# mitchelldurbincs/GeneralsReinforcementLearning

Measured on AMD Instinct MI355X. Metric: env steps/sec (whole node), 20x20 4P fog-on; state bit-exact vs the C restatement of the Go engine (the reference's own test vectors pass on both), higher is better.
Workload: dtype int32

## Files before the change

generalsreinforcementlearning_amd/csrc/gvec_device.hpp:

```cpp
#pragma once
#include <hip/hip_runtime.h>
#include <stdint.h>

#include "../../include/generals_vec.h"

extern "C" __device__ int gvec_llvm_writelane(int value, int lane, int vdst_in) __asm("llvm.amdgcn.writelane.i32");

#ifndef GVEC_NT
#define GVEC_NT 14
#endif
#define GVEC_NT_MASK 2
#define GVEC_NT_PLANE 4
#define GVEC_NT_ARMY 8
#ifndef GVEC_SC1
#define GVEC_SC1 1
#endif

namespace gvec {

typedef uint32_t u32x4 __attribute__((ext_vector_type(4)));

template <typename T>
__device__ __forceinline__ T ld_stream(const T* p) {
  if constexpr ((GVEC_NT & 1) != 0) return __builtin_nontemporal_load(p);
  return *p;
}
__device__ __forceinline__ void st_through(uint32_t* p, uint32_t v) { asm volatile("global_store_dword %0, %1, off sc1 nt" : : "v"(p), "v"(v) : "memory"); }
__device__ __forceinline__ void st_through(uint16_t* p, uint16_t v) {
  asm volatile("global_store_short %0, %1, off sc1 nt" : : "v"(p), "v"((uint32_t)v) : "memory");
}
__device__ __forceinline__ void st_through(float* p, float v) { asm volatile("global_store_dword %0, %1, off sc1 nt" : : "v"(p), "v"(v) : "memory"); }
__device__ __forceinline__ void st_through(u32x4* p, u32x4 v) {
  asm volatile("global_store_dwordx4 %0, %1, off sc1 nt\n\ts_nop 1" : : "v"(p), "v"(v) : "memory");
}
template <int CLASS, typename T>
__device__ __forceinline__ void st_stream(T* p, T v) {
  if constexpr ((GVEC_NT & CLASS) != 0) {
    if constexpr (GVEC_SC1 != 0) st_through(p, v);
    else __builtin_nontemporal_store(v, p);
  } else {
    *p = v;
  }
}

constexpr int HDR_DW = 24;
enum : int {
  H_TURN = 0,
  H_DIMS = 1,
  H_STATUS = 2,
  H_EPISODE = 3,
  H_ARMYCNT = 4,
  H_GIDX = 12,
  H_RECIPW = 20,
  H_CNT_STEPS = 21,
  H_CNT_ABORT = 22,
  H_CNT_DONE = 23
};
constexpr uint32_t HF_DONE = 1u, HF_FOG = 2u, HF_WIDE = 4u;
constexpr uint32_t HF_SETUP = 8u;
constexpr uint32_t HF_SYNC = 16u;
constexpr uint32_t HF_VSMALL = 32u;
constexpr uint32_t HF_LDIFF = 128u;
constexpr uint32_t HF_FEWSPECIAL = 64u;

template <int MAXP>
struct Planes {
  static constexpr int OWN = 0, VIS = MAXP, CHG = 2 * MAXP, VCH = 2 * MAXP + 1, GT1 = 2 * MAXP + 2,
                       GEN = 2 * MAXP + 3, CITY = 2 * MAXP + 4, MTN = 2 * MAXP + 5, VALID = 2 * MAXP + 6, NCOL0 = 2 * MAXP + 7,
                       NCOLL = 2 * MAXP + 8, OK = 2 * MAXP + 9 , LST = 2 * MAXP + 13,
                       COUNT = 3 * MAXP + 13, MUTABLE = 2 * MAXP + 3, SHARED = 13 ;
};

constexpr uint32_t KF_AGENT = 1u;
constexpr uint32_t KF_EMIT = 2u;
constexpr uint32_t KF_AUTORESET = 4u;
constexpr uint32_t KF_LMVALID = 16u;

struct StepArgs {
  uint32_t* hdr;
  uint32_t* rows;
  uint32_t* army16;
  int32_t* army32;
  const gvec_action* actions;
  gvec_action* actions_out;
  int32_t* err;
  uint32_t* legal;
  const uint32_t* zeros;
  const uint32_t* pool_hdr;
  const uint32_t* pool_rows;
  const uint32_t* pool_army16;
  const int32_t* pool_army32;
  int32_t num_envs, fd, row_dw, mask_dw, pool_size;
  int32_t pstride;
  int32_t prod_general, prod_city, prod_normal, interval;
  uint32_t interval_magic;
  int32_t turns, invalid_permille;
  uint32_t agent_noop, agent_half;
  uint32_t flags, seed_lo, seed_hi, pool_seed_lo, pool_seed_hi;
  uint32_t seed_base, pool_seed_base;
  int32_t env_base;
};

struct ArmyRef {
  uint32_t* n;
  int32_t* w;
};
struct ArmyCRef {
  const uint32_t* n;
  const int32_t* w;
  __device__ __forceinline__ ArmyCRef(const uint32_t* n_, const int32_t* w_) : n(n_), w(w_) {}
  __device__ __forceinline__ ArmyCRef(const ArmyRef& r) : n(r.n), w(r.w) {}
};
template <int NSLOT>
__device__ __forceinline__ ArmyRef army_ref(uint32_t* a16, int32_t* a32, int env) {
  return ArmyRef{a16 + (size_t)env * (NSLOT * 32), a32 + (size_t)env * (NSLOT * 64)};
}
template <int NSLOT>
__device__ __forceinline__ ArmyCRef army_cref(const uint32_t* a16, const int32_t* a32, int env) {
  return ArmyCRef(a16 + (size_t)env * (NSLOT * 32), a32 + (size_t)env * (NSLOT * 64));
}
template <int NSLOT>
__device__ __forceinline__ void army_load_narrow(int32_t (&army)[NSLOT], const uint32_t* n) {
  const int lane = (int)(threadIdx.x & 63u);
#pragma unroll
  for (int k = 0; k < NSLOT / 2; ++k) {
    const uint32_t w = ld_stream(n + 64 * k + lane);
    army[2 * k] = (int32_t)(w & 0xFFFFu);
    army[2 * k + 1] = (int32_t)(w >> 16);
  }
  if constexpr ((NSLOT & 1) != 0) army[NSLOT - 1] = (int32_t)ld_stream(reinterpret_cast<const uint16_t*>(n + 64 * (NSLOT / 2)) + lane);
}
template <int NSLOT>
__device__ __forceinline__ void army_load_wide(int32_t (&army)[NSLOT], const int32_t* w) {
  const int lane = (int)(threadIdx.x & 63u);
#pragma unroll
  for (int s = 0; s < NSLOT; ++s) army[s] = w[64 * s + lane];
}
template <int NSLOT>
__device__ __forceinline__ bool army_fits_narrow(const int32_t (&army)[NSLOT]) {
  uint32_t m = 0u;
#pragma unroll
  for (int s = 0; s < NSLOT; ++s) m |= (uint32_t)army[s];
  return __builtin_amdgcn_ballot_w64(m > 0xFFFFu) == 0ull;
}
template <int NSLOT>
__device__ __forceinline__ void army_store_narrow(const int32_t (&army)[NSLOT], uint32_t* n) {
  const int lane = (int)(threadIdx.x & 63u);
#pragma unroll
  for (int k = 0; k < NSLOT / 2; ++k) st_stream<GVEC_NT_ARMY>(n + 64 * k + lane, (uint32_t)army[2 * k] | ((uint32_t)army[2 * k + 1] << 16));
  if constexpr ((NSLOT & 1) != 0) st_stream<GVEC_NT_ARMY>(reinterpret_cast<uint16_t*>(n + 64 * (NSLOT / 2)) + lane, (uint16_t)army[NSLOT - 1]);
}
template <int NSLOT>
__device__ __forceinline__ void army_store_wide(const int32_t (&army)[NSLOT], int32_t* w) {
  const int lane = (int)(threadIdx.x & 63u);
#pragma unroll
  for (int s = 0; s < NSLOT; ++s) w[64 * s + lane] = army[s];
}

__device__ __forceinline__ int lane_id() { return (int)(threadIdx.x & 63u); }

template <int CTRL, int RM = 0xf, int BM = 0xf>
__device__ __forceinline__ uint32_t dpp0(uint32_t v) {
  return (uint32_t)__builtin_amdgcn_update_dpp(0, (int)v, CTRL, RM, BM, false);
}
__device__ __forceinline__ uint32_t from_prev(uint32_t v) { return dpp0<0x138>(v); }
__device__ __forceinline__ uint32_t from_next(uint32_t v) { return dpp0<0x130>(v); }

__device__ __forceinline__ uint32_t wave_scan_add(uint32_t v) {
// ... 233 lines not shown
```

generalsreinforcementlearning_amd/csrc/gvec_kernels.hip:

```cpp
#include "gvec_launch.hpp"
#include "gvec_packed.hpp"

#include <type_traits>

namespace gvec {

constexpr int WAVES_PER_BLOCK = 4;
#ifdef GYM_PLAYERS_WAVES
#define GYM_PLAYERS_WAVES_OF(NSLOT) GYM_PLAYERS_WAVES
#else
#define GYM_PLAYERS_WAVES_OF(NSLOT) ((NSLOT) <= 7 ? 4 : 3)
#endif

template <int MAXP, int NSLOT>
using Turn = PBoard<MAXP, NSLOT>;

template <int MAXP, int NSLOT>
__device__ __forceinline__ uint32_t agent_sample(const Turn<MAXP, NSLOT>& b, const uint32_t (&m)[Turn<MAXP, NSLOT>::NR][4], uint32_t ek,
                                                 const StepArgs& A) {
  using T = Turn<MAXP, NSLOT>;
  constexpr int NR = T::NR, PPR = T::PPR, ROWL = T::ROWL;
  const int lane = lane_id();
  const uint32_t sbase = ek + (uint32_t)b.turn * 0x9E3779B1u + 0x165667B1u;
  uint32_t mine = 0u;
#pragma unroll
  for (int k = 0; k < NR; ++k) {
    const uint32_t player = (uint32_t)T::lane_player(k);
    const uint32_t h1 = amix(mad24(player, 0x4A7C15u, sbase));
    const uint32_t h2 = amix(h1 ^ 0x68E31DA4u);
    const uint32_t hi16 = h2 >> 16;
    const bool act = b.lane_flag(b.alive, k) && !((h1 & 0xFFFFu) < A.agent_noop);
    const bool half = (h1 >> 16) < A.agent_half;
    const bool inv = A.invalid_permille > 0 && (__umul24(h2 & 0xFFFFu, 1000u) >> 16) < (uint32_t)A.invalid_permille;
    const uint32_t c0 = (uint32_t)__builtin_popcount(m[k][0]), c1 = c0 + (uint32_t)__builtin_popcount(m[k][1]);
    const uint32_t c2 = c1 + (uint32_t)__builtin_popcount(m[k][2]), cnt = c2 + (uint32_t)__builtin_popcount(m[k][3]);
    const uint32_t sc = row_scan_add<ROWL>(cnt);
    const uint32_t total = row_last<ROWL>(sc);
    const uint32_t kk = __umul24(hi16, total) >> 16;
    const uint32_t below = sc - cnt;
    const bool sel = kk >= below && kk < sc;
    const uint32_t r = kk - below;
    const uint32_t d = (r >= c0 ? 1u : 0u) + (r >= c1 ? 1u : 0u) + (r >= c2 ? 1u : 0u);
    const uint32_t base = (d == 0u) ? 0u : (d == 1u) ? c0 : (d == 2u) ? c1 : c2;
    const uint32_t w = (d == 0u) ? m[k][0] : (d == 1u) ? m[k][1] : (d == 2u) ? m[k][2] : m[k][3];
    const uint32_t t_sel = 32u * (uint32_t)T::col() + kth_set_bit(w, r - base);
    const uint32_t pick = row_scan_or<ROWL>(sel ? (t_sel | (d << 10) | 0x8000u) : 0u);
    const uint32_t unchecked = (__umul24(hi16, (uint32_t)b.N) >> 16) | (((h1 >> 8) & 3u) << 10) | 0x8000u;
    const uint32_t fin = inv ? unchecked : pick;
    const bool go = act && (fin & 0x8000u) != 0u;
    const uint32_t out = (fin & 0xFFFu) | (go ? 0x1000u : 0u) | (half ? 0x2000u : 0u);
    const uint32_t got = bperm((((lane % PPR) * ROWL) + ROWL - 1) << 2, out);
    mine = (lane / PPR == k) ? got : mine;
  }
  return mine;
}

template <int MAXP, int NSLOT>
__device__ __forceinline__ void agent_words(const Turn<MAXP, NSLOT>& b, uint32_t mine, uint32_t& alo, uint32_t& ahi) {
  const bool act = lane_id() < MAXP && (mine & 0x1000u) != 0u;
  const int t = (int)(mine & 0x3FFu), d = (int)((mine >> 10) & 3u);
  const int y = (int)(__umul24((uint32_t)t, (uint32_t)b.recipW) >> 16), x = t - (int)__umul24((uint32_t)y, (uint32_t)b.W);
  const int dx = (d == 1) - (d == 3), dy = (d == 2) - (d == 0);
  const uint32_t lo = ((uint32_t)x & 0xFFu) | (((uint32_t)y & 0xFFu) << 8) | (((uint32_t)(x + dx) & 0xFFu) << 16) |
                      (((uint32_t)(y + dy) & 0xFFu) << 24);
  alo = act ? lo : 0u;
  ahi = act ? (GVEC_ACT_VALID | ((mine & 0x2000u) ? GVEC_ACT_HALF : 0u)) : 0u;
}

template <int MAXP, int NSLOT>
__device__ __forceinline__ typename Turn<MAXP, NSLOT>::ActVec agent_actvec(const Turn<MAXP, NSLOT>& b, uint32_t mine, bool may_be_unchecked) {
  typename Turn<MAXP, NSLOT>::ActVec v;
  const bool act = lane_id() < MAXP && (mine & 0x1000u) != 0u;
  const int t = (int)(mine & 0x3FFu), d = (int)((mine >> 10) & 3u);
  uint32_t code = 0u;
  if (may_be_unchecked) {
    const int y = (int)(__umul24((uint32_t)t, (uint32_t)b.recipW) >> 16), x = t - (int)__umul24((uint32_t)y, (uint32_t)b.W);
    const bool off = (d == 0) ? (y == 0) : (d == 1) ? (x == b.W - 1) : (d == 2) ? (y == b.H - 1) : (x == 0);
    code = off ? GVEC_ERR_INVALID_COORDINATES : 0u;
  }
  v.meta = act ? (code | 16u | ((mine & 0x2000u) ? 32u : 0u)) : 0u;
  v.ft = t;
  v.tt = t + ((d == 0) ? -b.W : (d == 1) ? 1 : (d == 2) ? b.W : -1);
  return v;
}

template <typename BT>
__device__ __forceinline__ void load_board(BT& b, const uint32_t* hdr, const uint32_t* rows, const ArmyCRef& army, int fd) {
  b.load_hdr(hdr);
  b.load_army(army);
  b.load_planes(rows, fd);
}
template <bool EARLY = false, typename BT>
__device__ __forceinline__ void load_turn(BT& b, const uint32_t* hdr, const uint32_t* rows, const ArmyCRef& army, int fd, const uint32_t* zeros) {
  if constexpr (EARLY) {
    b.issue_hdr(hdr);
    b.load_planes(rows, fd, zeros);
    b.load_army_narrow(army);
    b.decode_hdr_scalar(hdr);
    b.land();
    b.land_scalars();
    b.spread_shared();
    b.load_lists(rows, fd);
    b.load_army_wide_if_flagged(army);
  } else {
    b.load_hdr(hdr);
    b.load_army(army);
    b.template load_planes<false>(rows, fd, zeros);
  }
}

template <int MAXP, int NSLOT, typename BT>
__device__ __forceinline__ void redeal(BT& b, const StepArgs& A, int env, int fd, int row_dw) {
  const uint32_t episode = b.hdr_get(H_EPISODE) + 1u;
  const uint32_t cs = b.hdr_get(H_CNT_STEPS), ca = b.hdr_get(H_CNT_ABORT), cd = b.hdr_get(H_CNT_DONE);
  const uint32_t hk = fmix32(env_key_of(A.pool_seed_base, (uint32_t)env) ^ (episode * 0x9E3779B1u));
  const int j = (int)__umulhi(hk, (uint32_t)A.pool_size);
  load_turn(b, A.pool_hdr + (size_t)j * HDR_DW, A.pool_rows + (size_t)j * row_dw, army_cref<NSLOT>(A.pool_army16, A.pool_army32, j), fd, A.zeros);
  b.hdr_set(H_EPISODE, episode);
  b.hdr_set(H_CNT_STEPS, cs);
  b.hdr_set(H_CNT_ABORT, ca);
  b.hdr_set(H_CNT_DONE, cd);
}

constexpr int step_waves(int maxp, int nslot) {
  const int ppr = (nslot <= 7) ? 4 : 2;
  const int nr = (maxp + ppr - 1) / ppr;
  const int state = 3 * nr + 13 + nr + nslot + 4 * nr;
  const int need = state + (state + 32 <= 62 ? 32 : 40);
  const int alloc = (need + 7) / 8 * 8;
  const int w = 512 / alloc;
  return w > 8 ? 8 : (w < 2 ? 2 : w);
}

template <int MAXP, int NSLOT, bool AGENT, bool ODD>
__global__ __launch_bounds__(64 * WAVES_PER_BLOCK, step_waves(MAXP, NSLOT)) void step_kernel(StepArgs A) {
  constexpr int FD = 2 * NSLOT - (ODD ? 1 : 0);
  constexpr int ROW_DW = (Planes<MAXP>::COUNT * FD + 3) / 4 * 4;
  __shared__ int32_t army_shadow[WAVES_PER_BLOCK][NSLOT * 64];
  using B = Turn<MAXP, NSLOT>;
  __shared__ uint32_t act_scratch[WAVES_PER_BLOCK][B::ACT_SCRATCH_DW];
  const int wave = (int)(threadIdx.x >> 6), lane = lane_id();
  const int env = uni((int)blockIdx.x * WAVES_PER_BLOCK + wave);
  if (env >= A.num_envs) return;
  bool force_redeal = false;
  if constexpr (!AGENT) {
    const uint32_t f0 = (uint32_t)uni((int)reinterpret_cast<const uint32_t*>(A.actions)[((size_t)env * A.pstride) * 2 + 1]);
    if (f0 & GVEC_ACT_SKIP_ENV) {
      if (A.err && lane == 0) A.err[env] = 0;
      return;
    }
    force_redeal = (f0 & GVEC_ACT_RESET_ENV) != 0u;
  }
  B b;
  b.larmy = army_shadow[wave];
  b.lscr = act_scratch[wave];
  const ArmyRef army_env = army_ref<NSLOT>(A.army16, A.army32, env);
  load_turn<true>(b, A.hdr + (size_t)env * HDR_DW, A.rows + (size_t)env * ROW_DW, army_env, FD, A.zeros);
  b.small = !(b.hflags & HF_WIDE);
  const bool emit = (A.flags & KF_EMIT) != 0u;
  uint32_t m[B::NR][4];
  uint32_t err = 0u;
  bool types_dirty = false, changed = true;
  const bool can_redeal = (A.flags & KF_AUTORESET) && A.pool_size > 0;
  if (AGENT && A.actions_out && (b.hflags & HF_DONE)) {
    if (lane < A.pstride) reinterpret_cast<uint2*>(A.actions_out)[(size_t)env * A.pstride + lane] = make_uint2(0u, 0u);
  }
  if (can_redeal && ((b.hflags & HF_DONE) || force_redeal)) {
    redeal<MAXP, NSLOT>(b, A, env, FD, ROW_DW);
    types_dirty = true;
  } else if (b.hflags & HF_DONE) {
    err = GVEC_ERR_GAME_OVER;
    changed = false;
  } else {
    typename B::ActVec av;
    if constexpr (AGENT) {
      b.template legal_planes<false>(m);
      uint32_t mine = (GVEC_PROFILE_SKIP & 1) ? 0u : agent_sample<MAXP, NSLOT>(b, m, env_key_of(A.seed_base, (uint32_t)env), A);
      if (GVEC_PROFILE_DUP & 64) { b.opaque(); b.template legal_planes<false>(m); }
      if (GVEC_PROFILE_DUP & 1) {
        b.opaque();
#pragma unroll
        for (int d = 0; d < 4; ++d) asm volatile("" : "+v"(m[0][d]));
        const uint32_t again = agent_sample<MAXP, NSLOT>(b, m, env_key_of(A.seed_base, (uint32_t)env), A);
        asm volatile("" : : "v"(again));
      }
      av = agent_actvec<MAXP, NSLOT>(b, mine, A.invalid_permille > 0);
      if (A.actions_out) {
        uint32_t alo, ahi;
        agent_words<MAXP, NSLOT>(b, mine, alo, ahi);
        if (lane < A.pstride) reinterpret_cast<uint2*>(A.actions_out)[(size_t)env * A.pstride + lane] = make_uint2(alo, ahi);
      }
    } else {
      uint32_t alo = 0u, ahi = 0u;
      if (lane < A.pstride) {
        const uint2 w = reinterpret_cast<const uint2*>(A.actions)[(size_t)env * A.pstride + lane];
        alo = w.x;
        ahi = w.y;
      }
      av = b.prevalidate(alo, ahi);
    }
    bool aborted;
    err = b.turn_step(av, A, aborted);
    if (!(GVEC_PROFILE_SKIP & 32)) b.refresh_gt1();
    if (GVEC_PROFILE_DUP & 32) { b.opaque_v(); b.refresh_gt1(); }
    b.hdr_set(H_CNT_STEPS, b.hdr_get(H_CNT_STEPS) + 1u);
    if (aborted) b.hdr_set(H_CNT_ABORT, b.hdr_get(H_CNT_ABORT) + 1u);
    if (b.hflags & HF_DONE) b.hdr_set(H_CNT_DONE, b.hdr_get(H_CNT_DONE) + 1u);
  }
  b.store_army_staged(army_env);
  b.settle_lists();
  b.store_hdr(A.hdr + (size_t)env * HDR_DW, err);
  if (types_dirty) b.store_planes(A.rows + (size_t)env * ROW_DW, FD, ROW_DW, true);
  else b.store_planes_staged(A.rows + (size_t)env * ROW_DW, FD);
  if (A.err && lane == 0) A.err[env] = (int32_t)err;
  if (!(GVEC_PROFILE_SKIP & 64) && emit && (changed || !(A.flags & KF_LMVALID))) {
    b.template legal_planes<false>(m);
    b.store_masks_staged(m, A.legal + (size_t)env * A.pstride * A.mask_dw, FD, A.pstride);
  }
}

constexpr int rollout_waves(int maxp, int nslot) {
  const int ppr = (nslot <= 7) ? 4 : 2;
  const int nr = (maxp + ppr - 1) / ppr;
  const int need = 3 * nr + 13 + nr + nslot + 4 * nr + (nslot >= 16 ? 100 : nslot >= 10 ? 68 : 44);
  const int alloc = (need + 7) / 8 * 8;
  const int w = 512 / alloc;
  return w > 8 ? 8 : (w < 2 ? 2 : w);
}

template <int MAXP, int NSLOT>
__global__ __launch_bounds__(64 * WAVES_PER_BLOCK, rollout_waves(MAXP, NSLOT)) void rollout_kernel(StepArgs A) {
  __shared__ int32_t army_shadow[WAVES_PER_BLOCK][NSLOT * 64];
  using B = Turn<MAXP, NSLOT>;
  __shared__ uint32_t act_scratch[WAVES_PER_BLOCK][B::ACT_SCRATCH_DW];
  const int wave = (int)(threadIdx.x >> 6), lane = lane_id();
  const int env = uni((int)blockIdx.x * WAVES_PER_BLOCK + wave);
  if (env >= A.num_envs) return;
  B b;
  b.larmy = army_shadow[wave];
  b.lscr = act_scratch[wave];
  const ArmyRef army_env = army_ref<NSLOT>(A.army16, A.army32, env);
  load_turn(b, A.hdr + (size_t)env * HDR_DW, A.rows + (size_t)env * A.row_dw, army_env, A.fd, A.zeros);
  uint32_t m[B::NR][4];
  uint32_t err = 0u, n_steps = 0u, n_abort = 0u, n_done = 0u;
  const uint32_t ek = env_key_of(A.seed_base, (uint32_t)env);
  const bool can_redeal = (A.flags & KF_AUTORESET) && A.pool_size > 0;
  int k = 0;
  for (;;) {
    b.template legal_planes<false>(m);
    while (k < A.turns && !(b.hflags & HF_DONE)) {
      const uint32_t mine = agent_sample<MAXP, NSLOT>(b, m, ek, A);
      bool aborted;
      err = b.turn_step(agent_actvec<MAXP, NSLOT>(b, mine, A.invalid_permille > 0), A, aborted);
      n_steps += 1u;
      n_abort += aborted ? 1u : 0u;
      n_done += (b.hflags & HF_DONE) ? 1u : 0u;
      ++k;
      b.refresh_gt1();
      b.template legal_planes<false>(m);
    }
    if (k >= A.turns) break;
    if (!can_redeal) {
      err = GVEC_ERR_GAME_OVER;
      break;
    }
    redeal<MAXP, NSLOT>(b, A, env, A.fd, A.row_dw);
    err = 0u;
    ++k;
  }
  b.hdr_set(H_CNT_STEPS, b.hdr_get(H_CNT_STEPS) + n_steps);
  b.hdr_set(H_CNT_ABORT, b.hdr_get(H_CNT_ABORT) + n_abort);
  b.hdr_set(H_CNT_DONE, b.hdr_get(H_CNT_DONE) + n_done);
  b.store_army(army_env);
  b.settle_lists();
  b.store_hdr(A.hdr + (size_t)env * HDR_DW, err);
  b.store_planes(A.rows + (size_t)env * A.row_dw, A.fd, A.row_dw, true);
  if (A.err && lane == 0) A.err[env] = (int32_t)err;
  b.store_masks_staged(m, A.legal + (size_t)env * A.pstride * A.mask_dw, A.fd, A.pstride);
}

template <int MAXP, int NSLOT, int MODE>
__global__ __launch_bounds__(64 * WAVES_PER_BLOCK) void query_kernel(StepArgs A) {
  using B = Turn<MAXP, NSLOT>;
  const int wave = (int)(threadIdx.x >> 6), lane = lane_id();
  const int env = uni((int)blockIdx.x * WAVES_PER_BLOCK + wave);
  if (env >= A.num_envs) return;
  B b;
  b.larmy = nullptr;
  load_turn(b, A.hdr + (size_t)env * HDR_DW, A.rows + (size_t)env * A.row_dw, army_cref<NSLOT>(A.army16, A.army32, env), A.fd, A.zeros);
  uint32_t m[B::NR][4];
  if constexpr (MODE == 2) b.template legal_planes<true>(m);
  else b.template legal_planes<false>(m);
  if constexpr (MODE == 1) {
    uint32_t alo = 0u, ahi = 0u;
    if (!(b.hflags & HF_DONE)) agent_words<MAXP, NSLOT>(b, agent_sample<MAXP, NSLOT>(b, m, env_key_of(A.seed_base, (uint32_t)env), A), alo, ahi);
    if (lane < A.pstride) reinterpret_cast<uint2*>(A.actions_out)[(size_t)env * A.pstride + lane] = make_uint2(alo, ahi);
  } else {
    b.store_masks(m, A.legal + (size_t)env * A.pstride * A.mask_dw, A.fd, A.pstride);
  }
}


__device__ __forceinline__ uint32_t bot_mix_draw(uint32_t ek, uint32_t turn, uint32_t player) {
  const uint32_t h = amix((ek ^ 0x5851F42Du) + turn * 0x2C1B3C6Du + player * 0x297A2D39u);
  return amix(h ^ 0x1B873593u);
}

__device__ __forceinline__ uint64_t wave_max_u64(uint64_t v) {
  const int lane = lane_id();
#pragma unroll
  for (int off = 32; off >= 1; off >>= 1) {
    const int src = (lane ^ off) << 2;
    const uint64_t o = ((uint64_t)bperm(src, (uint32_t)(v >> 32)) << 32) | bperm(src, (uint32_t)v);
    v = o > v ? o : v;
  }
  return v;
}

template <typename BT>
__device__ __forceinline__ bool row_any(uint32_t x) {
  const unsigned long long bal = __builtin_amdgcn_ballot_w64(x != 0u);
  return ((bal >> (BT::row() * BT::ROWL)) & (BT::ROWL == 32 ? 0xFFFFFFFFull : 0xFFFFull)) != 0ull;
}

template <typename BT>
__device__ __forceinline__ uint32_t rows_to_bits(bool flag, int k) {
  const unsigned long long bal = __builtin_amdgcn_ballot_w64(flag);
  uint32_t bits = 0u;
#pragma unroll
  for (int r = 0; r < BT::PPR; ++r)
    if ((bal >> (r * BT::ROWL)) & (BT::ROWL == 32 ? 0xFFFFFFFFull : 0xFFFFull)) bits |= 1u << (k * BT::PPR + r);
  return bits;
}

template <typename BT>
__device__ __forceinline__ uint32_t from_dir(const BT& b, uint32_t x, int d) {
  return d == 0 ? b.upW(x) : d == 1 ? b.dn1(x) : d == 2 ? b.dnW(x) : b.up1(x);
}

template <int MAXP, int NSLOT>
__global__ __launch_bounds__(64 * WAVES_PER_BLOCK) void bot_kernel(StepArgs A, BotArgs G) {
  using B = Turn<MAXP, NSLOT>;
  constexpr int NR = B::NR, PPR = B::PPR, ROWL = B::ROWL;
  __shared__ int32_t army_shadow[WAVES_PER_BLOCK][NSLOT * 64];
  const int wave = (int)(threadIdx.x >> 6), lane = lane_id();
  const int env = uni((int)blockIdx.x * WAVES_PER_BLOCK + wave);
  if (env >= A.num_envs) return;
  B b;
  b.larmy = &army_shadow[wave][0];
  load_turn(b, A.hdr + (size_t)env * HDR_DW, A.rows + (size_t)env * A.row_dw, army_cref<NSLOT>(A.army16, A.army32, env), A.fd, A.zeros);
  uint32_t m[NR][4];
  b.template legal_planes<false>(m);
  const bool done = (b.hflags & HF_DONE) != 0u;
  const uint32_t ek = env_key_of(A.seed_base, (uint32_t)env);

  uint32_t agent_mine = 0u, rnd_bits = 0u;
  if (G.random_permille > 0) {
    agent_mine = agent_sample<MAXP, NSLOT>(b, m, ek, A);
    const uint32_t h = bot_mix_draw(ek, (uint32_t)b.turn, (uint32_t)lane);
    const bool rnd = lane < MAXP && (__umul24(h & 0xFFFFu, 1000u) >> 16) < (uint32_t)G.random_permille;
    rnd_bits = (uint32_t)__builtin_amdgcn_ballot_w64(rnd);
  }
  const uint32_t movers = done ? 0u : (G.players & b.alive & ~rnd_bits);

  uint32_t bot_mine = 0u;
  if (movers != 0u) {
    const bool fog = (b.hflags & HF_FOG) != 0u;
    b.army_to_lds();
    uint32_t mok[4];
#pragma unroll
// ... 2312 lines not shown
```

generalsreinforcementlearning_amd/csrc/gvec_packed.hpp:

```cpp
#pragma once
#include "gvec_device.hpp"

#ifndef GVEC_PROFILE_SKIP
#define GVEC_PROFILE_SKIP 0
#endif
#ifndef GVEC_PROFILE_DUP
#define GVEC_PROFILE_DUP 0
#endif
#ifndef GVEC_ACT_VECTOR
#define GVEC_ACT_VECTOR 1
#endif

namespace gvec {

template <int ROWL>
__device__ __forceinline__ uint32_t row_scan_add(uint32_t v) {
  v += dpp0<0x111>(v);
  v += dpp0<0x112>(v);
  v += dpp0<0x114>(v);
  v += dpp0<0x118>(v);
  if constexpr (ROWL == 32) v += dpp0<0x142, 0xa>(v);
  return v;
}
template <int ROWL>
// ... 624 lines not shown
    atomicOr(cand ? &s_cand[fcol] : s_dummy, fbit);
    atomicOr(cand ? &s_cand[tcol] : s_dummy, tbit);
    wave_lds_fence();
    const int distinct = (int)rdlane(row_scan_add<ROWL>((uint32_t)__builtin_popcount(s_cand[lane & (ROWL - 1)])), ROWL - 1);
    const int ncand = __builtin_popcountll(__builtin_amdgcn_ballot_w64(cand));
    if (distinct != 2 * ncand) return false;
    const int32_t fa = larmy[ft], ta = larmy[tt];
    const int myrow = (lane % PPR) * ROWL;
    uint32_t w_ft = 0u;
#pragma unroll
    for (int k = 0; k < NR; ++k) {
      const uint32_t g = bperm((myrow + fcol) << 2, own[k]);
      w_ft = (lane / PPR == k) ? g : w_ft;
    }
    uint32_t owner_bits = 0u;
#pragma unroll
    for (int q = 0; q < MAXP; ++q) {
      const uint32_t g = bperm((((q % PPR) * ROWL) + tcol) << 2, own[q / PPR]);
      owner_bits |= ((g >> (tt & 31)) & 1u) << q;
    }
    const bool own_ft = ((w_ft >> (ft & 31)) & 1u) != 0u;
    const bool mine_tt = ((owner_bits >> lane) & 1u) != 0u;
    const bool mtn_tt = ((bperm(tcol << 2, mtn) >> (tt & 31)) & 1u) != 0u;
    const bool gen_tt = ((bperm(tcol << 2, gen) >> (tt & 31)) & 1u) != 0u;
    uint32_t dyn = mtn_tt ? GVEC_ERR_TARGET_IS_MOUNTAIN : 0u;
    dyn = (fa <= 1) ? GVEC_ERR_INSUFFICIENT_ARMY : dyn;
    dyn = own_ft ? dyn : GVEC_ERR_NOT_OWNED;
    const uint32_t code = cand ? dyn : scode;
    const bool ok = cand && dyn == 0u;
    {
      const unsigned long long em = __builtin_amdgcn_ballot_w64(active && code != 0u);
      if (em && !first_err) first_err = rdlane(code, (int)__builtin_ctzll(em));
    }
    int32_t n = (m & 32u) ? (fa >> 1) : (fa - 1);
    n = n < 1 ? 1 : n;
    const bool take = !mine_tt && n > ta;
    const bool capture = ok && take;
    const int32_t fight = take ? n - ta : ta - n;
    const int32_t new_ta = mine_tt ? ta + n : fight;
    larmy_store(ok ? &larmy[ft] : reinterpret_cast<int32_t*>(s_dummy), fa - n);
    larmy_store(ok ? &larmy[tt] : reinterpret_cast<int32_t*>(s_dummy), new_ta);
    atomicOr(ok ? &s_chg[fcol] : s_dummy, fbit);
    atomicOr(ok ? &s_chg[tcol] : s_dummy, tbit);
    atomicOr(capture ? &s_cap[tcol] : s_dummy, tbit);
    atomicOr(capture ? &s_own[64 * (lane / PPR) + myrow + tcol] : s_dummy, tbit);
    const int32_t burnt = take ? ta : n;
    const int32_t loss = (ok && !mine_tt) ? burnt : 0;
    atomicAdd((loss != 0 && owner_bits != 0u) ? &s_loss[__builtin_ctz(owner_bits | 0x80000000u) & 7] : s_dummy, (uint32_t)loss);
    wave_lds_fence();
    move_delta = -(loss + (int32_t)s_loss[lane & 7]);
    const uint32_t capbits = s_cap[col()];
    chg |= s_chg[col()];
    vch |= capbits;
#pragma unroll
    for (int k = 0; k < NR; ++k) own[k] = (own[k] & ~capbits) | s_own[64 * k + lane];
    unsigned long long el = __builtin_amdgcn_ballot_w64(capture && gen_tt);
    if (el) el = __builtin_amdgcn_ballot_w64(capture && gen_tt && owner_bits != 0u);
    while (el) {
      const int p = (int)__builtin_ctzll(el);
      el &= el - 1ull;
      const int prev = (int)__builtin_ctz(rdlane(owner_bits, p));
      if (!((elim_seen >> prev) & 1u)) {
        orders |= (uint64_t)((uint32_t)prev | ((uint32_t)p << 4)) << (8 * n_orders);
        n_orders++;
        elim_seen |= 1u << prev;
      }
    }
    return true;
  }

  template <int PID>
  __device__ __forceinline__ void act_chain(const ActVec& av, uint32_t& first_err, uint64_t& orders, int& n_orders,
                                            uint32_t& elim_seen) {
    if constexpr (PID < MAXP) {
      if (PID < P) apply_action<PID>(av, first_err, orders, n_orders, elim_seen);
      act_chain<PID + 1>(av, first_err, orders, n_orders, elim_seen);
    }
  }

  __device__ __forceinline__ void eliminate(uint64_t orders, int n_orders) {
    for (int e = 0; e < n_orders; ++e) {
      const int v = (int)((orders >> (8 * e)) & 15u), nw = (int)((orders >> (8 * e + 4)) & 15u);
      uint32_t tiles = 0u;
#pragma unroll
      for (int k = 0; k < NR; ++k) tiles |= (lane_player(k) == v) ? (lst[k] & own[k]) : 0u;
      tiles = or_rows(tiles);
#pragma unroll
      for (int k = 0; k < NR; ++k) {
        own[k] = (lane_player(k) == v) ? (own[k] & ~tiles) : own[k];
        own[k] = (lane_player(k) == nw) ? (own[k] | tiles) : own[k];
      }
      hdr_set(H_GIDX + v, 0xFFFFFFFFu);
      chg |= tiles;
      vch |= tiles;
      hflags &= ~HF_VSMALL;
      alive &= ~(1u << v);
    }
  }

  __device__ __forceinline__ uint32_t turn_step(uint32_t acts_lo, uint32_t acts_hi, const StepArgs& A, bool& aborted) {
    return turn_step(prevalidate(acts_lo, acts_hi), A, aborted);
  }
  __device__ __forceinline__ uint32_t turn_step(const ActVec& av, const StepArgs& A, bool& aborted) {
    aborted = false;
    turn++;
    const bool matched = lists_match();
    if (!(GVEC_PROFILE_SKIP & 2)) update_fog(matched);
    if (GVEC_PROFILE_DUP & 2) { opaque(); update_fog(matched); }
    chg = 0u;
    vch = 0u;
    hflags |= HF_VSMALL;
    bool delta = matched && (hflags & HF_SYNC) != 0u;
    move_delta = 0;
    uint32_t first_err = 0u, elim_seen = 0u;
    uint64_t orders = 0ull;
    int n_orders = 0;
    const unsigned long long present = __builtin_amdgcn_ballot_w64((av.meta & 16u) != 0u && lane_id() < P);
    if (present && !(GVEC_PROFILE_SKIP & 4)) {
      army_to_lds();
      if (!(GVEC_ACT_VECTOR && lscr && act_vector(av, first_err, orders, n_orders, elim_seen))) {
        act_chain<0>(av, first_err, orders, n_orders, elim_seen);
        delta = false;
      }
      army_from_lds();
    }
    if (n_orders > 0) {
      eliminate(orders, n_orders);
      update_stats();
    }
    if (first_err) {
      if (n_orders == 0) hflags &= ~HF_SYNC;
      aborted = true;
      return first_err;
    }
    if (!(GVEC_PROFILE_SKIP & 8)) production(A.prod_general, A.prod_city, A.prod_normal, A.interval, A.interval_magic);
    if (!(GVEC_PROFILE_SKIP & 16)) update_stats(n_orders == 0, delta && n_orders == 0);
    if (GVEC_PROFILE_DUP & 16) { opaque_v(); update_stats(n_orders == 0, false); }
    check_game_over();
    return 0u;
  }

  __device__ __forceinline__ void initial_setup() {
    turn = 0;
    chg = 0u;
    vch = 0u;
#pragma unroll
    for (int k = 0; k < NR; ++k) vis[k] = 0u;
    hflags = (hflags & ~HF_DONE) | HF_VSMALL;
    update_stats();
    update_fog();
    check_game_over();
  }

  template <bool SERIALIZER = false>
  __device__ __forceinline__ void legal_planes(uint32_t (&m)[NR][4]) const {
#pragma unroll
    for (int k = 0; k < NR; ++k) {
      const uint32_t s = SERIALIZER ? (own[k] & gt1) : (lst[k] & own[k] & gt1);
      const uint32_t src = (SERIALIZER || lane_flag(alive, k)) ? s : 0u;
      m[k][0] = src & ok[0];
      m[k][1] = src & (SERIALIZER ? ok[2] : ok[1]);
      m[k][2] = src & (SERIALIZER ? ok[3] : ok[2]);
      m[k][3] = src & (SERIALIZER ? ok[1] : ok[3]);
    }
  }
  __device__ __forceinline__ void store_masks(const uint32_t (&m)[NR][4], uint32_t* legal_env, int fd, int pstride) const {
    const bool in = col() < fd;
#pragma unroll
    for (int k = 0; k < NR; ++k) {
      const int p = lane_player(k);
      if (in && p < pstride && p < MAXP) {
        uint32_t* g = legal_env + (size_t)p * (4 * fd) + col();
#pragma unroll
        for (int d = 0; d < 4; ++d) st_stream<GVEC_NT_MASK>(g + d * fd, m[k][d]);
      }
    }
  }
  template <int CLASS>
  __device__ __forceinline__ void flush_stage(uint32_t* dst, int dwords) const {
    const u32x4* s4 = reinterpret_cast<const u32x4*>(larmy);
    u32x4* g4 = reinterpret_cast<u32x4*>(dst);
    const int chunks = dwords >> 2;
    for (int i = lane_id(); i < chunks; i += 64) {
      st_stream<CLASS>(g4 + i, s4[i]);
    }
    const int tail = dwords & 3, l = lane_id();
    if (l < tail) st_stream<CLASS>(dst + 4 * chunks + l, reinterpret_cast<const uint32_t*>(larmy)[4 * chunks + l]);
  }
  __device__ __forceinline__ void store_planes_staged(uint32_t* rows_env, int fd) const {
    uint32_t* stage = reinterpret_cast<uint32_t*>(larmy);
    const bool in = col() < fd;
    uint32_t* g = stage + row() * fd + col();
    wave_lds_fence();
#pragma unroll
    for (int k = 0; k < NR; ++k) {
      if (in && (k * PPR + row() < MAXP)) {
        g[(PL::OWN + k * PPR) * fd] = own[k];
        g[(PL::VIS + k * PPR) * fd] = vis[k];
      }
    }
#pragma unroll
    for (int k = 0; k * PPR < 3; ++k) {
      const int j = k * PPR + row();
      if (in && j < 3) g[(PL::CHG + k * PPR) * fd] = j == 0 ? chg : (j == 1 ? vch : gt1);
    }
    wave_lds_fence();
    flush_stage<GVEC_NT_PLANE>(rows_env, PL::MUTABLE * fd);
    store_lists(rows_env, fd);
  }
  __device__ __forceinline__ void store_army_narrow_staged(uint32_t* n) const {
    uint32_t* stage = reinterpret_cast<uint32_t*>(larmy);
    const int lane = lane_id();
    wave_lds_fence();
#pragma unroll
    for (int k = 0; k < NSLOT / 2; ++k) stage[64 * k + lane] = (uint32_t)army[2 * k] | ((uint32_t)army[2 * k + 1] << 16);
    if constexpr ((NSLOT & 1) != 0) reinterpret_cast<uint16_t*>(stage + 64 * (NSLOT / 2))[lane] = (uint16_t)army[NSLOT - 1];
    wave_lds_fence();
    flush_stage<GVEC_NT_ARMY>(n, NSLOT * 32);
  }
  __device__ __forceinline__ void store_army_staged(const ArmyRef& a) {
    if (army_fits_narrow<NSLOT>(army)) {
      hflags &= ~HF_WIDE;
      store_army_narrow_staged(a.n);
    } else {
      hflags |= HF_WIDE;
      army_store_wide<NSLOT>(army, a.w);
    }
  }
  __device__ __forceinline__ void store_masks_staged(const uint32_t (&m)[NR][4], uint32_t* legal_env, int fd, int pstride) const {
    static_assert(MAXP <= 8, "the army shadow holds the mask block");
    if ((reinterpret_cast<uintptr_t>(legal_env) & 15u) != 0u) {
      store_masks(m, legal_env, fd, pstride);
      return;
    }
    uint32_t* stage = reinterpret_cast<uint32_t*>(larmy);
    const bool in = col() < fd;
    wave_lds_fence();
#pragma unroll
    for (int k = 0; k < NR; ++k) {
      const int p = lane_player(k);
      if (in && p < pstride && p < MAXP) {
        uint32_t* g = stage + p * (4 * fd) + col();
#pragma unroll
        for (int d = 0; d < 4; ++d) g[d * fd] = m[k][d];
      }
    }
    wave_lds_fence();
    flush_stage<GVEC_NT_MASK>(legal_env, pstride * 4 * fd);
  }
};

}
```

Measured before the change: 1.202 billion.

## Skip global stores of unchanged ownership, visibility and legal-mask planes

Keeps a per-lane snapshot of the owner, visibility and legal-source bits right after the turn loads. At store time, the plane flush skips the owner and visibility ranges when they are unchanged. The mask flush stores a chunk only when some ballot over rows shows a source bit changed. This cuts write traffic for steps where these planes stay the same, at the cost of extra registers, ballots and branch logic in the store path. Skipping is turned off when the wide or list-diff flags are set or the types were rewritten.

```diff
diff --git a/generalsreinforcementlearning_amd/csrc/gvec_device.hpp b/generalsreinforcementlearning_amd/csrc/gvec_device.hpp
--- a/generalsreinforcementlearning_amd/csrc/gvec_device.hpp
+++ b/generalsreinforcementlearning_amd/csrc/gvec_device.hpp
@@ -14,6 +14,10 @@
 #define GVEC_NT_ARMY 8
 #ifndef GVEC_SC1
 #define GVEC_SC1 1
+#endif
+
+#ifndef GVEC_STORE_SKIP
+#define GVEC_STORE_SKIP 1
 #endif
 
 namespace gvec {
diff --git a/generalsreinforcementlearning_amd/csrc/gvec_kernels.hip b/generalsreinforcementlearning_amd/csrc/gvec_kernels.hip
--- a/generalsreinforcementlearning_amd/csrc/gvec_kernels.hip
+++ b/generalsreinforcementlearning_amd/csrc/gvec_kernels.hip
@@ -157,6 +157,9 @@
   const ArmyRef army_env = army_ref<NSLOT>(A.army16, A.army32, env);
   load_turn<true>(b, A.hdr + (size_t)env * HDR_DW, A.rows + (size_t)env * ROW_DW, army_env, FD, A.zeros);
   b.small = !(b.hflags & HF_WIDE);
+  typename B::Kept kept;
+  if constexpr (GVEC_STORE_SKIP != 0) b.keep(kept);
+  const typename B::Kept* const same = (GVEC_STORE_SKIP != 0) ? &kept : nullptr;
   const bool emit = (A.flags & KF_EMIT) != 0u;
   uint32_t m[B::NR][4];
   uint32_t err = 0u;
@@ -211,11 +214,12 @@
   b.settle_lists();
   b.store_hdr(A.hdr + (size_t)env * HDR_DW, err);
   if (types_dirty) b.store_planes(A.rows + (size_t)env * ROW_DW, FD, ROW_DW, true);
-  else b.store_planes_staged(A.rows + (size_t)env * ROW_DW, FD);
+  else b.store_planes_staged(A.rows + (size_t)env * ROW_DW, FD, same);
   if (A.err && lane == 0) A.err[env] = (int32_t)err;
   if (!(GVEC_PROFILE_SKIP & 64) && emit && (changed || !(A.flags & KF_LMVALID))) {
     b.template legal_planes<false>(m);
-    b.store_masks_staged(m, A.legal + (size_t)env * A.pstride * A.mask_dw, FD, A.pstride);
+    const bool masks_current = (A.flags & KF_LMVALID) != 0u && !types_dirty;
+    b.store_masks_staged(m, A.legal + (size_t)env * A.pstride * A.mask_dw, FD, A.pstride, masks_current ? same : nullptr);
   }
 }
 
diff --git a/generalsreinforcementlearning_amd/csrc/gvec_packed.hpp b/generalsreinforcementlearning_amd/csrc/gvec_packed.hpp
--- a/generalsreinforcementlearning_amd/csrc/gvec_packed.hpp
+++ b/generalsreinforcementlearning_amd/csrc/gvec_packed.hpp
@@ -800,12 +800,12 @@
     check_game_over();
   }
 
+  __device__ __forceinline__ uint32_t legal_src(int k) const { return lane_flag(alive, k) ? (lst[k] & own[k] & gt1) : 0u; }
   template <bool SERIALIZER = false>
   __device__ __forceinline__ void legal_planes(uint32_t (&m)[NR][4]) const {
 #pragma unroll
     for (int k = 0; k < NR; ++k) {
-      const uint32_t s = SERIALIZER ? (own[k] & gt1) : (lst[k] & own[k] & gt1);
-      const uint32_t src = (SERIALIZER || lane_flag(alive, k)) ? s : 0u;
+      const uint32_t src = SERIALIZER ? (own[k] & gt1) : legal_src(k);
       m[k][0] = src & ok[0];
       m[k][1] = src & (SERIALIZER ? ok[2] : ok[1]);
       m[k][2] = src & (SERIALIZER ? ok[3] : ok[2]);
@@ -825,17 +825,47 @@
     }
   }
   template <int CLASS>
-  __device__ __forceinline__ void flush_stage(uint32_t* dst, int dwords) const {
+  __device__ __forceinline__ void flush_stage(uint32_t* dst, int dwords, int same_lo = 0, int same_hi = 0) const {
     const u32x4* s4 = reinterpret_cast<const u32x4*>(larmy);
     u32x4* g4 = reinterpret_cast<u32x4*>(dst);
     const int chunks = dwords >> 2;
     for (int i = lane_id(); i < chunks; i += 64) {
+      if (4 * i >= same_lo && 4 * i + 4 <= same_hi) continue;
       st_stream<CLASS>(g4 + i, s4[i]);
     }
     const int tail = dwords & 3, l = lane_id();
     if (l < tail) st_stream<CLASS>(dst + 4 * chunks + l, reinterpret_cast<const uint32_t*>(larmy)[4 * chunks + l]);
   }
-  __device__ __forceinline__ void store_planes_staged(uint32_t* rows_env, int fd) const {
+  struct Kept {
+    uint32_t own[NR], vis[NR];
+    uint32_t src[NR];
+    bool plain;
+  };
+  __device__ __forceinline__ void keep(Kept& z) const {
+#pragma unroll
+    for (int k = 0; k < NR; ++k) {
+      z.own[k] = own[k];
+      z.vis[k] = vis[k];
+      z.src[k] = legal_src(k);
+    }
+    z.plain = !(hflags & (HF_WIDE | HF_LDIFF));
+  }
+  __device__ __forceinline__ bool may_skip(const Kept& z) const { return z.plain && !(hflags & (HF_WIDE | HF_LDIFF)); }
+
+  __device__ __forceinline__ void store_planes_staged(uint32_t* rows_env, int fd, const Kept* z = nullptr) const {
+    int same_lo = 0, same_hi = 0;
+    if (z) {
+      uint32_t d_own = 0u, d_vis = 0u;
+#pragma unroll
+      for (int k = 0; k < NR; ++k) {
+        d_own |= own[k] ^ z->own[k];
+        d_vis |= vis[k] ^ z->vis[k];
+      }
+      static_assert(PL::OWN == 0 && PL::VIS == MAXP, "the unchanged run is one range of the block's head");
+      const bool skip = may_skip(*z);
+      same_lo = (skip && !any_bit(d_own)) ? 0 : PL::VIS * fd;
+      same_hi = (skip && !any_bit(d_vis)) ? PL::CHG * fd : PL::VIS * fd;
+    }
     uint32_t* stage = reinterpret_cast<uint32_t*>(larmy);
     const bool in = col() < fd;
     uint32_t* g = stage + row() * fd + col();
@@ -853,7 +883,7 @@
       if (in && j < 3) g[(PL::CHG + k * PPR) * fd] = j == 0 ? chg : (j == 1 ? vch : gt1);
     }
     wave_lds_fence();
-    flush_stage<GVEC_NT_PLANE>(rows_env, PL::MUTABLE * fd);
+    flush_stage<GVEC_NT_PLANE>(rows_env, PL::MUTABLE * fd, same_lo, same_hi);
     store_lists(rows_env, fd);
   }
   __device__ __forceinline__ void store_army_narrow_staged(uint32_t* n) const {
@@ -875,7 +905,8 @@
       army_store_wide<NSLOT>(army, a.w);
     }
   }
-  __device__ __forceinline__ void store_masks_staged(const uint32_t (&m)[NR][4], uint32_t* legal_env, int fd, int pstride) const {
+  __device__ __forceinline__ void store_masks_staged(const uint32_t (&m)[NR][4], uint32_t* legal_env, int fd, int pstride,
+                                                     const Kept* z = nullptr) const {
     static_assert(MAXP <= 8, "the army shadow holds the mask block");
     if ((reinterpret_cast<uintptr_t>(legal_env) & 15u) != 0u) {
       store_masks(m, legal_env, fd, pstride);
@@ -894,7 +925,33 @@
       }
     }
     wave_lds_fence();
-    flush_stage<GVEC_NT_MASK>(legal_env, pstride * 4 * fd);
+    if (!z) {
+      flush_stage<GVEC_NT_MASK>(legal_env, pstride * 4 * fd);
+      return;
+    }
+    const bool skip = may_skip(*z);
+    uint32_t ch_lo[NR], ch_hi[NR];
+#pragma unroll
+    for (int k = 0; k < NR; ++k) {
+      const unsigned long long c = skip ? __builtin_amdgcn_ballot_w64(legal_src(k) != z->src[k]) : ~0ull;
+      ch_lo[k] = (uint32_t)c;
+      ch_hi[k] = (uint32_t)(c >> 32);
+    }
+    const u32x4* s4 = reinterpret_cast<const u32x4*>(larmy);
+    u32x4* g4 = reinterpret_cast<u32x4*>(legal_env);
+    const int chunks = pstride * fd;
+    const uint32_t recip_fd = (uint32_t)((65536 + fd - 1) / fd);
+    for (int i = lane_id(); i < chunks; i += 64) {
+      const int p = (int)(__umul24((uint32_t)i, recip_fd) >> 16);
+      const int sh = (p % PPR) * ROWL;
+      uint32_t mine = 0u;
+#pragma unroll
+      for (int k = 0; k < NR; ++k) {
+        const uint32_t half = (sh & 32) ? ch_hi[k] : ch_lo[k];
+        mine = (p / PPR == k) ? half : mine;
+      }
+      if (((mine >> (sh & 31)) & (ROWL == 32 ? 0xFFFFFFFFu : 0xFFFFu)) != 0u) st_stream<GVEC_NT_MASK>(g4 + i, s4[i]);
+    }
   }
 };
 
```

Result: no change. 1.212 billion (median of 6 runs) (+0.8%).
